# 2alaaa/distributed-llm-scheduler

Hardware: AMD Instinct MI355X
Metric: DAG makespan (ms) + tasks completed under mem cap, GPT-2 DAG at 1/2/4/8 MI355X (lower is better)
Workload: dtype bf16

## Files before the change

csrc/kernels/gemm_glds_impl.h:

```cpp
#pragma once
#include <cstdlib>
#include <type_traits>
#include "common.h"
#include "kernels.h"
#include "gemm_glds_cfgs.h"

#ifndef DLS_STAMP
#define DLS_STAMP(k)
#endif

namespace {

__device__ __forceinline__ int kslice_count(int K, int kslice) { return K / kslice; }

template <int N>
__device__ __forceinline__ void wait_vm() {
  asm volatile("s_waitcnt vmcnt(%0)" ::"n"(N) : "memory");
}
template <int PW, int A>
__device__ __forceinline__ void wait_tiles(int ahead) {
  if constexpr (A == 0) {
    wait_vm<0>();
  } else {
    if (ahead >= A) wait_vm<PW * A>();
    else wait_tiles<PW, A - 1>(ahead);
  }
}
__device__ __forceinline__ void raw_barrier() { asm volatile("s_barrier" ::: "memory"); }
template <class T>
__device__ __forceinline__ void consume_from_here(T& x) {
  asm volatile("" : "+v"(x));
}
template <bool WAIT_LDS_ONLY>
__device__ __forceinline__ void epi_barrier() {
  if constexpr (WAIT_LDS_ONLY) asm volatile("s_waitcnt lgkmcnt(0)\n\ts_barrier" ::: "memory");
  else __syncthreads();
}

template <int BM_, int BN_, int WM_, int WN_, int STAGES_, int PRIO_ = 0, int BXS_ = 0, int KG_ = 1, int RING_ = 0,
          int OCC_ = 1>
struct Cfg {
  static constexpr int BM = BM_, BN = BN_, WM = WM_, WN = WN_, STAGES = STAGES_, PRIO = PRIO_, BXS = BXS_;
  static constexpr int KG = KG_, RING = RING_, OCC = OCC_;
  static constexpr int BK = 64, CH = 8;
  static constexpr int NW = WM * WN, T = 64 * NW * KG;
  static constexpr int WTM = BM / WM, WTN = BN / WN, FM = WTM / 16, FN = WTN / 16;
  static constexpr bool HALF_FRAGS = FM + FN > 12;
  static constexpr int ROWS = BM + BN, INSTR = ROWS / 8, PW = (INSTR + NW - 1) / NW;
  static constexpr int SUB = ROWS * CH;
  static constexpr int STAGE = SUB * KG;
  static constexpr int SA = STAGES, SB = STAGES + BXS;
  static constexpr int PWA = (BM / 8 + NW - 1) / NW, PWB = (BN / 8 + NW - 1) / NW;
  static constexpr bool EVEN = INSTR % NW == 0, EVEN_A = (BM / 8) % NW == 0, EVEN_B = (BN / 8) % NW == 0;
  static constexpr int A_STAGE = BM * CH, B_STAGE = BN * CH;
  static constexpr int LDS_UNITS = BXS ? SA * A_STAGE + SB * B_STAGE : STAGES * STAGE;
  static_assert(BM % 8 == 0 && BN % 8 == 0, "DMA pieces are 8 rows");
  static_assert(FM >= 1 && FN >= 1, "wave tile too small");
  static_assert(PW * (STAGES - 2) <= 63, "vmcnt range");
  static_assert(!BXS || (SA - 2) * PWA + (SA - 1) * PWB <= 63, "vmcnt range (split rings)");
  static_assert(STAGES >= 2 && STAGES <= 8, "stages");
  static_assert(LDS_UNITS * 16 <= 163840, "LDS budget");
  static_assert(KG == 1 || (BXS == 0 && PRIO == 0), "K groups use the joint ring");
  static_assert(KG == 1 || (KG - 1) * NW * 64 * FM * FN * 16 <= LDS_UNITS * 16, "K-group reduction must fit the LDS");
  static constexpr bool EPI_BATCH = FM * FN <= 4;
// ... 647 lines not shown
          float csv[8] = {0.f, 0.f, 0.f, 0.f, 0.f, 0.f, 0.f, 0.f};
          if (bias) {
            uint32_t w[8];
            if (pre_bvec) {
#pragma unroll
              for (int h = 0; h < 2; ++h) {
                consume_from_here(o_bv[h]);
                const uint32_t p0 = o_bv[h][0], p1 = o_bv[h][1];
                w[4 * h + 0] = p0 << 16;
                w[4 * h + 1] = p0 & 0xffff0000u;
                w[4 * h + 2] = p1 << 16;
                w[4 * h + 3] = p1 & 0xffff0000u;
              }
            } else {
#pragma unroll
              for (int e = 0; e < 8; ++e) {
                consume_from_here(o_bs[e]);
                w[e] = o_bs[e] << 16;
              }
            }
#pragma unroll
            for (int e = 0; e < 8; ++e) bv[e] = col + e < N ? __uint_as_float(w[e]) : 0.f;
          }
          if constexpr (LNM) {
#pragma unroll
            for (int h = 0; h < 2; ++h) consume_from_here(o_cs[h]);
#pragma unroll
            for (int e = 0; e < 8; ++e) csv[e] = col + e < N ? __uint_as_float(o_cs[e >> 2][e & 3]) : 0.f;
          }
          float v[8];
#pragma unroll
          for (int e = 0; e < 8; ++e) {
            const float x = e < 4 ? lo[e & 3] : hi[e & 3];
            if constexpr (LNM) v[e] = act_c<ACT>(ln_rs1 * (x - ln_mu1 * csv[e]) + bv[e]);
            else v[e] = act_c<ACT>(alpha * x + bv[e]);
          }
          if constexpr (ROPE) {
            rope_pairs<4>(v, row, col, rope);
            rope_pairs<4>(v + 4, row, col + 4, rope);
          }
#pragma unroll
          for (int e = 0; e < 8; ++e) o[e] = f2bf(v[e]);
        };
        per_epilogue(finish);
        if (pre_res) consume_from_here(o_r);
        store_segment(o, rl, cc, o_r);
      }
      DLS_STAMP(3)
      return;
    }
  }
  if constexpr (C::EPI_BATCH) {
    if (part == nullptr && act != ACT_SWIGLU) request_operands();
  }
  if constexpr (C::KG > 2) {
    constexpr int REG = C::NW * C::FM * C::FN * 64;
    epi_barrier<C::EPI_BATCH>();
    f32x4* red = reinterpret_cast<f32x4*>(smem);
    if (kgrp != 0) {
#pragma unroll
      for (int i = 0; i < C::FM; ++i)
#pragma unroll
        for (int j = 0; j < C::FN; ++j)
          red[(kgrp - 1) * REG + ((i * C::FN + j) * C::NW + wq) * 64 + lane] = acc[i][j];
    }
    epi_barrier<C::EPI_BATCH>();
    if (kgrp == 0) {
#pragma unroll
// ... 612 lines not shown
  using type = Cfg<224, 256, 2, 4, 2, 0, 1>;
};
template <>
struct TallTile<C33> {
  using type = C14;
};

template <class C>
void grouped(const GemmArgs& a, int n_groups, const int* offsets, const unsigned long long* w_ptrs,
             const unsigned long long* c_ptrs, hipStream_t s, const int* a_rows) {
  static const int w_stream = [] {
    const char* e = std::getenv("DLS_EXPERT_NT");
    return e && e[0] == '0' ? 0 : 1;
  }();
  const char* pe = std::getenv("DLS_EXPERT_PAIRS");
  const int pairs = pe && *pe ? std::atoi(pe) : 2;
  const int pair = a.grouped_shared ? 0 : pairs;
  const char* xe = std::getenv("DLS_EXPERT_XCD");
  const bool xcd = xe && *xe == '1' && !a.grouped_shared && pair != 1;
  const char* te = std::getenv("DLS_EXPERT_TALL");
  const bool tall = !(te && *te == '0') && !a.grouped_shared;
  const Epi ep{a.rope, nullptr, nullptr, nullptr, w_ptrs, c_ptrs,
               (a.grouped_shared ? 8 : ((size_t)a.M * a.lda * 2 < (1ull << 31) ? w_stream : 0)) |
                   (pair == 1 ? 16 : pair == 2 ? 32 : pair == 3 ? 64 : 0) | (xcd ? 128 : 0) | (tall ? 256 : 0)};
  const int tiles_n = (a.N + C::BN - 1) / C::BN;
  const int blocks = pair == 1 ? (n_groups * tiles_n + 7) / 8 * 16 : pair >= 2 ? 2 * n_groups * tiles_n
                                                                               : n_groups * tiles_n;
  hipLaunchKernelGGL((gemm_glds_kernel<C, 0, 3>), dim3(blocks), dim3(C::T), 0, s, (const bf16*)a.A, a.lda,
                     nullptr, a.ldw, (bf16*)a.C, a.ldc, nullptr, nullptr, 0,
                     const_cast<float*>(reinterpret_cast<const float*>(a_rows)), a.M, a.N, a.K, a.act, a.alpha,
                     n_groups, tiles_n, 1, a.K, nullptr, 0, 1e-5f, offsets, a.compact_rows, ep);
}

template <int W_, int S_>
struct PrivCfg {
  static constexpr int W = W_, S = S_, BM = 32, BN = 48, BK = 64, CH = 8, FM = 2, FN = 3;
  static constexpr int T = 64 * W, PW = (BM + BN) / 8;
  static constexpr int SLOT = (BM + BN) * CH;
  static constexpr int RING = S * SLOT, LDS_UNITS = W * RING;
  static constexpr int REG = FM * FN * 64;
  static_assert(S >= 1 && PW * (S - 1) <= 63, "vmcnt range");
  static_assert(LDS_UNITS * 16 <= 163840 && T <= 1024, "LDS budget, block size");
  static_assert(REG <= RING, "a wave's fragment region lies inside its own ring");
  static_assert(T >= BM * 8, "one 16-byte output segment per storing thread");
};

template <class P>
__device__ __forceinline__ void mainloop_private(bf16x8* ring, const bf16* __restrict__ A, int lda,
                                                 const bf16* __restrict__ W, int ldw, int M, int N, int m0, int n0,
                                                 int kbeg, int nk, int lane, f32x4 (&acc)[P::FM][P::FN]) {
  const bf16* src[P::PW];
#pragma unroll
  for (int j = 0; j < P::PW; ++j) {
    const int row = 8 * j + (lane >> 3);
    const int kofs = kbeg + ((lane & 7) ^ (row & 7)) * 8;
    src[j] = row < P::BM ? A + (size_t)min(m0 + row, M - 1) * lda + kofs
                         : W + (size_t)min(n0 + row - P::BM, N - 1) * ldw + kofs;
  }
  auto issue = [&](int kt, bf16x8* slot) {
#pragma unroll
    for (int j = 0; j < P::PW; ++j)
      __builtin_amdgcn_global_load_lds((const void*)(src[j] + kt * P::BK),
                                       (__attribute__((address_space(3))) void*)(slot + j * 64), 16, 0, 0);
  };
#pragma unroll
  for (int s = 0; s < P::S; ++s)
    if (s < nk) issue(s, ring + s * P::SLOT);
  int sl = 0;
  for (int kt = 0; kt < nk; ++kt) {
    wait_tiles<P::PW, P::S - 1>(min(P::S - 1, nk - 1 - kt));
    bf16x8* slot = ring + sl * P::SLOT;
    const bf16x8* sA = slot;
    const bf16x8* sB = slot + P::BM * P::CH;
    bf16x8 af[2][P::FM], bw[2][P::FN];
#pragma unroll
    for (int kk = 0; kk < 2; ++kk) {
      const int chunk = kk * 4 + (lane >> 4);
#pragma unroll
      for (int j = 0; j < P::FN; ++j) {
        const int row = j * 16 + (lane & 15);
        bw[kk][j] = sB[row * P::CH + (chunk ^ (row & 7))];
      }
#pragma unroll
      for (int i = 0; i < P::FM; ++i) {
        const int row = i * 16 + (lane & 15);
        af[kk][i] = sA[row * P::CH + (chunk ^ (row & 7))];
      }
    }
    __builtin_amdgcn_sched_barrier(0);
    asm volatile("s_waitcnt lgkmcnt(0)" ::: "memory");
    __builtin_amdgcn_sched_barrier(0);
    if (kt + P::S < nk) issue(kt + P::S, slot);
    __builtin_amdgcn_sched_barrier(0);
#pragma unroll
    for (int kk = 0; kk < 2; ++kk)
#pragma unroll
      for (int i = 0; i < P::FM; ++i)
#pragma unroll
        for (int j = 0; j < P::FN; ++j) acc[i][j] = mfma16x16x32(bw[kk][j], af[kk][i], acc[i][j]);
    sl = sl + 1 == P::S ? 0 : sl + 1;
  }
}

template <class P, int SPOL>
__global__ __launch_bounds__(P::T, 1) void gemm_private_kernel(const bf16* __restrict__ A, int lda,
                                                               const bf16* __restrict__ W, int ldw,
                                                               bf16* __restrict__ Cp, int ldc,
                                                               const bf16* __restrict__ bias,
                                                               const bf16* __restrict__ R, int ldr,
                                                               float* __restrict__ stats_out, int M, int N, int K,
                                                               float alpha, int tiles_m) {
  __shared__ bf16x8 smem[P::LDS_UNITS];
  const int tid = threadIdx.x, lane = tid & 63;
  const int wave = __builtin_amdgcn_readfirstlane(tid >> 6);
  const int tile = xcd_remap(blockIdx.x, gridDim.x);
  const int m0 = (tile % tiles_m) * P::BM, n0 = (tile / tiles_m) * P::BN;
  DLS_STAMP(0)
  const int nk = K / (P::BK * P::W);
  bf16x8* ring = smem + wave * P::RING;
  f32x4 acc[P::FM][P::FN];
#pragma unroll
  for (int i = 0; i < P::FM; ++i)
#pragma unroll
    for (int j = 0; j < P::FN; ++j) acc[i][j] = f32x4{0.f, 0.f, 0.f, 0.f};
  mainloop_private<P>(ring, A, lda, W, ldw, M, N, m0, n0, wave * nk * P::BK, nk, lane, acc);
  DLS_STAMP(1)
  constexpr int BNC = P::BN / 8, BNP = 8;
  const bool own = tid < P::BM * BNP;
  const int rl = tid / BNP, cc = tid % BNP;
  const int row = m0 + rl, col = n0 + cc * 8;
  const bool pre_bvec = ((reinterpret_cast<uintptr_t>(bias) & 7) | (N & 3)) == 0;
  const bool v16 = ((reinterpret_cast<uintptr_t>(Cp) | ((uintptr_t)ldc * 2)) & 15) == 0 &&
                   (!R || ((reinterpret_cast<uintptr_t>(R) | ((uintptr_t)ldr * 2)) & 15) == 0);
  const bool pre_res = R != nullptr && N >= 8 && v16 && ((size_t)(M + P::BM) * ldr * 2 < (1ull << 31));
  u32x2 o_bv[2];
  u32x4 o_r;
  if (own) {
    constexpr int kRaw = 0x00020000;
    if (bias && pre_bvec) {
      const auto rs = __builtin_amdgcn_make_buffer_rsrc(const_cast<bf16*>(bias), 0, N * 2, kRaw);
#pragma unroll
      for (int h = 0; h < 2; ++h) o_bv[h] = __builtin_amdgcn_raw_buffer_load_b64(rs, col * 2 + h * 8, 0, 0);
    }
    if (pre_res) {
// ... 90 lines not shown
        s2 += __shfl_xor(s2, o_, 64);
      }
      if (cc == 0 && row < M) {
        atomicAdd(stats_out + 2 * row, s1);
        atomicAdd(stats_out + 2 * row + 1, s2);
      }
    }
  }
  DLS_STAMP(3)
}

inline bool private_takes(int waves, const GemmArgs& a, int splitk, bool folded_norm, bool ranged) {
  return waves > 0 && a.K > 0 && a.K % (64 * waves) == 0 && splitk <= 1 && !folded_norm && !ranged &&
         a.act == ACT_NONE && a.rope.cols == 0 && !a.ext_stats;
}

template <int W_, int S_>
void launch_private(const GemmArgs& a, hipStream_t s) {
  using P = PrivCfg<W_, S_>;
  const int tiles_m = (a.M + P::BM - 1) / P::BM, tiles_n = (a.N + P::BN - 1) / P::BN;
  dim3 grid(tiles_m * tiles_n), block(P::T);
#define DLS_PK(POL_)                                                                                               \
  hipLaunchKernelGGL((gemm_private_kernel<P, POL_>), grid, block, 0, s, (const bf16*)a.A, a.lda, (const bf16*)a.W, \
                     a.ldw, (bf16*)a.C, a.ldc, (const bf16*)a.bias, (const bf16*)a.R, a.ldr, a.stats_out, a.M, a.N, \
                     a.K, a.alpha, tiles_m)
  switch ((size_t)a.M * a.ldc * 2 < (1ull << 31) ? a.stream_pol & 7 : 0) {
    case 2: case 3: DLS_PK(kPolStream); break;
    case 4: case 5: DLS_PK(kPolWT); break;
    default: DLS_PK(0);
  }
#undef DLS_PK
}

}

#define DLS_GLDS_DEFINE(ID)                                                                                     \
  bool glds_launch_cfg##ID(const GemmArgs& a, int splitk, float* ws, hipStream_t s, const float* ln_colsum,     \
                           int ln_mode, float ln_eps, const int* rows, bool persist) {                          \
    return launch<C##ID>(a, splitk, ws, s, ln_colsum, ln_mode, ln_eps, rows, persist);                          \
  }                                                                                                             \
  void glds_grouped_cfg##ID(const GemmArgs& a, int n_groups, const int* offsets, const unsigned long long* w_ptrs, \
                            const unsigned long long* c_ptrs, hipStream_t s, const int* a_rows) {               \
    grouped<C##ID>(a, n_groups, offsets, w_ptrs, c_ptrs, s, a_rows);                                            \
  }
```

csrc/kernels/gemm_private.hip:

```cpp
#include "gemm_glds_impl.h"

namespace {
constexpr int kWaves[kGemmPrivateCount] = {8, 4, 6, 12};
}

int gemm_private_waves(int cfg) {
  return cfg >= kGemmPrivate && cfg < kGemmPrivate + kGemmPrivateCount ? kWaves[cfg - kGemmPrivate] : 0;
}

bool gemm_private_takes(const GemmArgs& a, int cfg, int splitk, bool folded_norm, bool ranged) {
  return private_takes(gemm_private_waves(cfg), a, splitk, folded_norm, ranged);
}

bool launch_gemm_private(const GemmArgs& a, int cfg, hipStream_t s) {
  if (!gemm_private_takes(a, cfg, 1, false, false)) return false;
  switch (cfg - kGemmPrivate) {
    case 0: launch_private<8, 2>(a, s); break;
    case 1: launch_private<4, 3>(a, s); break;
    case 2: launch_private<6, 2>(a, s); break;
    default: launch_private<12, 1>(a, s); break;
  }
  return true;
}
```

csrc/kernels/kernels.h:

```cpp
#pragma once

#include <hip/hip_runtime_api.h>
#include <stdint.h>

constexpr int kActSwiglu = 4;

struct RopeArgs {
  const float* cos = nullptr;
  const float* sin = nullptr;
  int S = 1, D = 2, cols = 0;
};

struct GemmArgs {
  const void* A;
  int lda;
  const void* W;
  int ldw;
  void* C;
  int ldc;
  const void* bias;
  const void* R;
  int ldr;
  int M, N, K;
  int act;
// ... 11 lines not shown
  int norm_mode = 0;
  float norm_eps = 1e-5f;
  int ldn = 0;
  int stream_pol = 0;
};

struct Epi {
  RopeArgs rope;
  float* stats_out;
  const float* ext_stats;
  int* tile_sem = nullptr;
  const unsigned long long* grp_w = nullptr;
  const unsigned long long* grp_c = nullptr;
  int w_stream = 0;
};

int gemm_pick_config(int M, int N, int K);
void launch_gemm_bf16(const GemmArgs& a, hipStream_t s);

int gemm_glds_num_configs();
int gemm_glds_kstep(int cfg);
void gemm_glds_tile(int cfg, int* bm, int* bn);
int gemm_glds_resolve(int cfg, int act, bool ln_in);
constexpr int kGemmPersist = 64;
void gemm_glds_pick(int M, int N, int K, int* cfg, int* splitk);
size_t gemm_glds_workspace_bytes(int M, int N, int splitk);
bool launch_gemm_glds(const GemmArgs& a, int cfg, int splitk, void* workspace, hipStream_t s,
                      const float* ln_colsum = nullptr, int ln_mode = 0, float ln_eps = 1e-5f,
                      const int* rows = nullptr);
constexpr int kGemmPrivate = 120, kGemmPrivateCount = 4;
int gemm_private_waves(int cfg);
bool gemm_private_takes(const GemmArgs& a, int cfg, int splitk, bool folded_norm, bool ranged);
bool launch_gemm_private(const GemmArgs& a, int cfg, hipStream_t s);

void launch_gemm_glds_grouped(const GemmArgs& a, int cfg, int n_groups, const int* offsets,
                              const unsigned long long* w_ptrs, const unsigned long long* c_ptrs, hipStream_t s,
                              const int* a_rows = nullptr);

struct GemmGroupedSkinnyArgs {
  const void* A;
  int lda;
  int a_total;
  const int* a_rows;
  const int* offsets;
  const unsigned long long* w_ptrs;
  const unsigned long long* c_ptrs;
  void* C;
  int ldc;
  int compact_rows;
  int R, N, K;
  int act;
  int n_groups;
};
bool gemm_grouped_skinny_takes(int N, int K, int act);
void launch_gemm_grouped_skinny(const GemmGroupedSkinnyArgs& a, hipStream_t s);

constexpr int kSkinnyMaxRows = 16;
struct GemmSkinnyArgs {
  const void* A;
  int lda;
  const void* W;
  int ldw;
  void* C;
  int ldc;
  const void* bias;
  const void* R;
// ... 350 lines not shown
```

csrc/kernels/ops_binding.cpp:

```cpp
#include <cstdlib>

#include <torch/extension.h>
#include <c10/hip/HIPStream.h>

#include "kernels.h"

namespace {

hipStream_t cur_stream() { return c10::hip::getCurrentHIPStream().stream(); }

constexpr int64_t kSemPool = 1 << 20;
int64_t sem_next[64];
int* split_k_counters(const at::Tensor& like, int64_t n) {
  static at::Tensor* pool = new at::Tensor[64];
  int64_t* next = sem_next;
  const int d = like.get_device();
  TORCH_CHECK(d >= 0 && d < 64 && n <= kSemPool, "split-K counters");
  if (!pool[d].defined()) pool[d] = at::zeros({kSemPool}, like.options().dtype(at::kInt));
  n = (n + 63) / 64 * 64;
  if (next[d] + n > kSemPool) next[d] = 0;
  int* p = pool[d].data_ptr<int>() + next[d];
  next[d] += n;
  return p;
}
// ... 10 lines not shown
  const int old = g_fixup_max_slices;
  if (n > 0) g_fixup_max_slices = (int)std::min<int64_t>(n, 1 << 30);
  return old;
}

void check_bf16(const at::Tensor& t, const char* name) {
  TORCH_CHECK(t.is_cuda(), name, " must be a GPU tensor");
  TORCH_CHECK(t.scalar_type() == at::kBFloat16, name, " must be bfloat16");
}

void check_rows(const at::Tensor& t, const char* name) {
  TORCH_CHECK(t.dim() == 2, name, " must be 2-D");
  TORCH_CHECK(t.stride(1) == 1, name, " must have contiguous rows");
  TORCH_CHECK(t.stride(0) % 8 == 0, name, " row stride must be a multiple of 8 elements");
  TORCH_CHECK(reinterpret_cast<uintptr_t>(t.data_ptr()) % 16 == 0, name, " must be 16-byte aligned");
}

at::Tensor as2d(const at::Tensor& t) { return t.dim() == 2 ? t : t.reshape({-1, t.size(-1)}); }

constexpr int64_t kRegStage = 100;

at::Tensor gemm(const at::Tensor& a_in, const at::Tensor& w, const c10::optional<at::Tensor>& bias,
                const c10::optional<at::Tensor>& residual, int64_t act, double alpha,
                const c10::optional<at::Tensor>& out, int64_t config, int64_t splitk,
                const c10::optional<at::Tensor>& ln_colsum, int64_t ln_mode, double ln_eps,
                const c10::optional<at::Tensor>& rows, bool compact_rows,
                const c10::optional<at::Tensor>& rope_cos, const c10::optional<at::Tensor>& rope_sin, int64_t rope_S,
                int64_t rope_D, int64_t rope_cols, const c10::optional<at::Tensor>& stats_out,
                const c10::optional<at::Tensor>& ext_stats, const c10::optional<at::Tensor>& norm_out,
                const c10::optional<at::Tensor>& norm_w, const c10::optional<at::Tensor>& norm_b, int64_t norm_mode,
                double norm_eps, int64_t stream_pol) {
  check_bf16(a_in, "A");
  check_bf16(w, "W");
  const bool priv = gemm_private_waves((int)config) != 0;
  TORCH_CHECK(config < kRegStage + 4 || priv, "unknown GEMM config ", config, " (register-staged configs are ",
              kRegStage, "..", kRegStage + 3, ", wave-private rings ", kGemmPrivate, "..",
              kGemmPrivate + kGemmPrivateCount - 1, ")");
  at::Tensor a = as2d(a_in);
  check_rows(a, "A");
  check_rows(w, "W");
  const int64_t M = a.size(0), K = a.size(1), N = w.size(0);
  const bool swiglu = act == kActSwiglu;
  const int64_t NO = swiglu ? N / 2 : N;
  TORCH_CHECK(w.size(1) == K, "W must be [N][K] with K = ", K, ", got ", w.sizes());
  TORCH_CHECK(K % 8 == 0, "K must be a multiple of 8");
  TORCH_CHECK(!swiglu || (N % 32 == 0 && K % 64 == 0 && !residual.has_value()),
              "SwiGLU epilogue needs N % 32 == 0, K % 64 == 0 and no residual");
  at::Tensor c;
  if (out.has_value()) {
    c = as2d(*out);
    check_bf16(c, "out");
    TORCH_CHECK((c.size(0) == M || (compact_rows && c.size(0) <= M)) && c.size(1) == NO && c.stride(1) == 1,
                "out must be [M][N_out] (or fewer rows with compact_rows)");
  } else {
    c = at::empty({M, NO}, a.options());
  }
  const void* bptr = nullptr;
  if (bias.has_value()) {
    check_bf16(*bias, "bias");
    TORCH_CHECK(bias->is_contiguous() && bias->numel() == N, "bias must be contiguous [N]");
    bptr = bias->data_ptr();
  }
  const void* rptr = nullptr;
  int ldr = 0;
  if (residual.has_value()) {
    at::Tensor r = as2d(*residual);
    check_bf16(r, "residual");
    TORCH_CHECK(r.size(0) == M && r.size(1) == N && r.stride(1) == 1, "residual must be [M][N]");
    rptr = r.data_ptr();
    ldr = (int)r.stride(0);
// ... 35 lines not shown
    if (norm_mode == 2)
      launch_rmsnorm(c.data_ptr(), nullptr, nullptr, g.norm_w, y_n.data_ptr(), (int)M, (int)N, (float)norm_eps,
                     cur_stream());
    else
      launch_layernorm(c.data_ptr(), nullptr, nullptr, g.norm_w, g.norm_b, y_n.data_ptr(), (int)M, (int)N,
                       (float)norm_eps, cur_stream());
  };
  TORCH_CHECK(!compact_rows || (rows.has_value() && !residual.has_value()), "compact_rows needs rows and no residual");
  auto check_stats = [&](const at::Tensor& t, const char* name) {
    TORCH_CHECK(t.is_cuda() && t.scalar_type() == at::kFloat && t.is_contiguous() && t.numel() == 2 * M, name,
                " must be a contiguous fp32 [M][2] GPU tensor");
  };
  if (stats_out.has_value()) {
    check_stats(*stats_out, "stats_out");
    TORCH_CHECK(!swiglu && !rows.has_value(), "row statistics are emitted by plain (non-SwiGLU, full-row) GEMMs");
    g.stats_out = stats_out->data_ptr<float>();
  }
  if (ext_stats.has_value()) {
    check_stats(*ext_stats, "ext_stats");
    TORCH_CHECK(ln_mode != 0, "ext_stats needs ln_mode (1 LayerNorm, 2 RMSNorm) and ln_colsum");
    g.ext_stats = ext_stats->data_ptr<float>();
  }
  if (rope_cols > 0) {
    TORCH_CHECK(rope_cos.has_value() && rope_sin.has_value() && rope_cos->scalar_type() == at::kFloat &&
                    rope_sin->scalar_type() == at::kFloat && rope_cos->is_contiguous() && rope_sin->is_contiguous() &&
                    rope_cos->is_cuda() && rope_sin->is_cuda() &&
                    rope_cos->numel() >= rope_S * rope_D / 2 && rope_sin->numel() >= rope_S * rope_D / 2,
                "RoPE epilogue: cos/sin fp32 [S][D/2]");
    TORCH_CHECK(rope_D % 4 == 0 && rope_cols % rope_D == 0 && rope_cols <= N && !swiglu && K % 64 == 0 &&
                    !rows.has_value() && act == 0,
                "RoPE epilogue: D % 4 == 0, whole heads, LDS-DMA kernel, no activation / SwiGLU / row range");
    g.rope = RopeArgs{rope_cos->data_ptr<float>(), rope_sin->data_ptr<float>(), (int)rope_S, (int)rope_D,
                      (int)rope_cols};
    if (config >= kRegStage && !priv) config = -1;
  }
  const bool glds_ok = (K % 64 == 0);
  const float* csp = nullptr;
  if (ln_mode != 0) {
    TORCH_CHECK(glds_ok, "fused norm-GEMM needs K % 64 == 0");
    TORCH_CHECK(ln_colsum.has_value() && ln_colsum->scalar_type() == at::kFloat && ln_colsum->is_contiguous() &&
                    ln_colsum->numel() == N,
                "fused norm-GEMM needs fp32 ln_colsum [N]");
    csp = ln_colsum->data_ptr<float>();
  }
  if (priv) {
    TORCH_CHECK(!compact_rows && gemm_private_takes(g, (int)config, (int)splitk, ln_mode != 0, rowp != nullptr),
                "GEMM config ", config, " (wave-private rings, ", gemm_private_waves((int)config),
                " waves) takes plain launches only: K % ", 64 * gemm_private_waves((int)config),
                " == 0, no activation, folded norm, RoPE, SwiGLU, split-K or row range");
    TORCH_CHECK(launch_gemm_private(g, (int)config, cur_stream()), "GEMM config ", config, " refused the launch");
    post_norm(false);
    return c;
  }
  if (ln_mode != 0 || swiglu || rowp || stats_out.has_value()) {
    TORCH_CHECK(glds_ok, "this epilogue needs the LDS-DMA kernel (K % 64 == 0)");
    if (config >= kRegStage) config = -1;
  }
  if (config >= kRegStage || !glds_ok) {
    g.config = config >= kRegStage ? (int)(config - kRegStage) : -1;
    launch_gemm_bf16(g, cur_stream());
    post_norm(false);
    return c;
  }
  int cfg = (int)config, sk = (int)splitk;
  if (cfg < 0 || sk <= 0) {
    int acfg, ask;
    gemm_glds_pick((int)M, (int)N, (int)K, &acfg, &ask);
    if (cfg < 0) cfg = acfg;
    if (sk <= 0) sk = ask;
  }
  TORCH_CHECK((cfg & (kGemmPersist - 1)) < gemm_glds_num_configs() && cfg < 2 * kGemmPersist, "unknown GEMM config ", cfg);
  TORCH_CHECK(K % gemm_glds_kstep(cfg) == 0, "GEMM config ", cfg, " needs K % ", gemm_glds_kstep(cfg), " == 0");
  const bool split_ok = (N % 8 == 0) && (c.stride(0) % 8 == 0) && (ldr % 8 == 0) &&
                        K % (gemm_glds_kstep(cfg) * sk) == 0 &&
                        (!swiglu || N % 32 == 0);
  if (!split_ok || (ln_mode != 0 && !ext_stats.has_value())) sk = 1;
  at::Tensor ws;
  if (sk > 1) {
    ws = at::empty({(int64_t)gemm_glds_workspace_bytes((int)M, (int)N, sk) / 4}, a.options().dtype(at::kFloat));
    if (kSplitKFixup && sk <= g_fixup_max_slices && !rowp && !norm_out.has_value()) {
      int bm, bn;
      gemm_glds_tile(gemm_glds_resolve(cfg, (int)act, false), &bm, &bn);
      g.tile_sem = split_k_counters(a, (M + bm - 1) / bm * ((N + bn - 1) / bn));
// ... 1478 lines not shown
        py::arg("stats_out") = py::none(), py::arg("ext_stats") = py::none(), py::arg("norm_out") = py::none(),
        py::arg("norm_w") = py::none(), py::arg("norm_b") = py::none(), py::arg("norm_mode") = 0,
        py::arg("norm_eps") = 1e-5, py::arg("stream_pol") = 0);
  m.def("gemm_w8", &gemm_w8, py::arg("a"), py::arg("wq"), py::arg("scale"), py::arg("bias") = py::none(),
        py::arg("residual") = py::none(), py::arg("act") = 0, py::arg("alpha") = 1.0, py::arg("out") = py::none(),
        py::arg("config") = -1, py::arg("splitk") = 0, py::arg("store_pol") = 0, py::arg("workspace") = py::none());
  m.def("gemm_w8_num_configs", &gemm_w8_num_configs);
  m.def("gemm_w8_pick", [](int M, int N, int K) {
    int c, s;
    gemm_w8_pick(M, N, K, &c, &s);
    return std::make_pair(c, s);
  });
  m.def("gemm_grouped_w8", &gemm_grouped_w8, py::arg("x"), py::arg("weights"), py::arg("scales"), py::arg("w_ptrs"),
        py::arg("s_ptrs"), py::arg("offsets"), py::arg("act") = 0, py::arg("out") = py::none(),
        py::arg("outs") = std::vector<at::Tensor>{}, py::arg("out_ptrs") = py::none(), py::arg("config") = -1,
        py::arg("rows_hint") = 0, py::arg("a_rows") = py::none(), py::arg("shared_weights") = false,
        py::arg("store_pol") = 0);
  m.def("gemm_w8_grouped_num_configs", &gemm_w8_grouped_num_configs);
  m.def("gemm_w8_grouped_tile_rows", &gemm_w8_grouped_tile_rows);
  m.def("gemm_w8_grouped_pick", &gemm_w8_grouped_pick);
  m.def("gemm_grouped_w4a8", &gemm_grouped_w4a8, py::arg("xq"), py::arg("xscale"), py::arg("weights"),
        py::arg("scales"), py::arg("w_ptrs"), py::arg("s_ptrs"), py::arg("offsets"), py::arg("act") = 0,
        py::arg("out") = py::none(), py::arg("outs") = std::vector<at::Tensor>{}, py::arg("out_ptrs") = py::none(),
        py::arg("config") = -1, py::arg("rows_hint") = 0, py::arg("a_rows") = py::none(),
        py::arg("shared_weights") = false, py::arg("store_pol") = 0);
  m.def("gemm_w4a8_grouped_num_configs", &gemm_w4a8_grouped_num_configs);
  m.def("gemm_w4a8_grouped_tile_rows", &gemm_w4a8_grouped_tile_rows);
  m.def("gemm_w4a8_grouped_pick", &gemm_w4a8_grouped_pick);
  m.attr("REGSTAGE") = kRegStage;
  m.attr("PERSIST") = kGemmPersist;
  m.attr("PRIVATE") = kGemmPrivate;
  m.attr("PRIVATE_COUNT") = kGemmPrivateCount;
  m.def("gemm_private_waves", &gemm_private_waves);
  m.def("gemm_pick_config", &gemm_pick_config);
  m.def("gemm_glds_num_configs", &gemm_glds_num_configs);
  m.def("gemm_glds_kstep", &gemm_glds_kstep);
  m.def("gemm_glds_tile", [](int64_t cfg) {
    int bm, bn;
    gemm_glds_tile((int)cfg, &bm, &bn);
    return std::make_tuple((int64_t)bm, (int64_t)bn);
  });
  m.def("_split_k_cursor", &split_k_cursor);
  m.def("gemm_glds_pick", [](int M, int N, int K) {
    int c, s;
    gemm_glds_pick(M, N, K, &c, &s);
    return std::make_pair(c, s);
  });
  m.def("attention", &attention, py::arg("q"), py::arg("k"), py::arg("v"), py::arg("B"), py::arg("S"),
        py::arg("n_head"), py::arg("n_kv_head"), py::arg("head_dim"), py::arg("causal") = true,
        py::arg("scale") = 0.125, py::arg("out") = py::none(), py::arg("variant") = 0, py::arg("Sq") = 0,
        py::arg("q_off") = 0, py::arg("flags") = 0);
  m.def("kv_append", &kv_append, py::arg("k_new"), py::arg("v_new"), py::arg("k_cache"), py::arg("v_cache"),
        py::arg("pos"), py::arg("T"), py::arg("k_scale") = py::none(), py::arg("v_scale") = py::none());
  m.def("attention_decode_sizes", &attention_decode_sizes, py::arg("B"), py::arg("T"), py::arg("C"),
        py::arg("n_head"), py::arg("n_kv_head"), py::arg("head_dim"), py::arg("chunk") = 0);
  m.def("attention_decode_chunk", [](int64_t B, int64_t C, int64_t n_kv_head, int64_t head_dim) {
    return (int64_t)attn_decode_chunk((int)B, (int)C, (int)n_kv_head, (int)head_dim);
  });
  m.def("attention_decode", &attention_decode, py::arg("q"), py::arg("k_cache"), py::arg("v_cache"), py::arg("pos"),
        py::arg("T"), py::arg("n_head"), py::arg("n_kv_head"), py::arg("head_dim"), py::arg("scale"),
        py::arg("part"), py::arg("cnt"), py::arg("out") = py::none(), py::arg("chunk") = 0,
        py::arg("k_scale") = py::none(), py::arg("v_scale") = py::none());
  m.def("gemm_fixup_max_slices", &gemm_fixup_max_slices, py::arg("n") = 0);
  m.def("kv_dequantize_rows", &kv_dequantize_rows, py::arg("cache"), py::arg("scale"), py::arg("pos"), py::arg("T"),
        py::arg("out"));
  m.def("attention_chunk_variant", &attention_chunk_variant, py::arg("B"), py::arg("T"), py::arg("n_head"),
// ... 80 lines not shown
```

distributed_llm_scheduler_amd/ops/__init__.py:

```python
from __future__ import annotations

import math
import os
import threading
from typing import Optional, Tuple

import torch
import torch.nn.functional as F

from . import tuning

ACT = {None: 0, "none": 0, "gelu": 1, "gelu_tanh": 1, "silu": 2, "relu": 3, "swiglu": 4}
SWIGLU = 4
SWIGLU_BLOCK = 16
LMHEAD_POL = int(os.environ.get("DLS_LMHEAD_POL", "3"))
LMHEAD_MIN_N = 32000
WEIGHT_NT_MB = float(os.environ.get("DLS_WEIGHT_NT_MB", "0"))
ACT_POL = int(os.environ.get("DLS_ACT_POL", "4"))
ACT_POL_MODEL = {"mixtral-8x7b": 0}
_ACT_POL_SET = "DLS_ACT_POL" in os.environ
ATTN_FLAGS = int(os.environ.get("DLS_ATTN_FLAGS", "0"))
ATTN_VARIANT = int(os.environ.get("DLS_ATTN_VARIANT", "0"))


# ... 168 lines not shown
    return dict(norm_out=y, norm_w=nw, norm_b=nb if kind == "layernorm" else None,
                norm_mode=1 if kind == "layernorm" else 2, norm_eps=float(eps))


def _post_norm_ref(src, post_norm):
    y, nw, nb, kind, eps = post_norm
    s2 = src.reshape(-1, src.shape[-1])
    r = ref_layernorm(s2, nw, nb, eps) if kind == "layernorm" else ref_rmsnorm(s2, nw, eps)
    y.view(r.shape).copy_(r)


def linear(x, w, bias=None, act=None, residual=None, alpha=1.0, out=None, rows=None, rows_hint=None,
           compact=False, rope=None, stats_out=None, post_norm=None):
    a = ACT[act] if not isinstance(act, int) else act
    n_out = w.shape[0] // 2 if a == SWIGLU else w.shape[0]
    if _gpu(x):
        shp = x.shape[:-1] + (n_out,)
        M = x.numel() // x.shape[-1]
        cfg, sk = tuning.lookup(rows_hint or M, w.shape[0], w.shape[1], tuning.tag(a, rows is not None))
        if cfg == tuning.LIB:
            if tuning.VENDOR and a == 0 and residual is None and rows is None and rope is None \
                    and stats_out is None and post_norm is None:
                x2 = x.reshape(M, x.shape[-1])
                o2 = out.view(M, n_out) if out is not None else torch.empty(M, n_out, dtype=x.dtype, device=x.device)
                if bias is not None:
                    torch.addmm(bias, x2, w.t(), beta=1.0, alpha=float(alpha), out=o2)
                else:
                    torch.mm(x2, w.t(), out=o2)
                    if alpha != 1.0:
                        o2.mul_(alpha)
                return o2.view(shp) if out is None else out
            cfg, sk = tuning.lookup_fused(rows_hint or M, w.shape[0], w.shape[1], tuning.tag(a, rows is not None))
        cfg, sk = tuning.resolve_private((cfg, sk), w.shape[1], a, rows is not None, rope is not None)
        rc, rs_, rS, rD, rcols = rope if rope is not None else (None, None, 1, 2, 0)
        y = ext().gemm(x, w, bias, residual, a, float(alpha), out, cfg, sk, None, 0, 1e-5, rows, bool(compact),
                       rc, rs_, int(rS), int(rD), int(rcols), stats_out, None,
                       stream_pol=_stream_pol(w.shape[0], w.shape[1]) if rows is None else 0,
                       **(_post_norm_args(post_norm) if post_norm is not None else {}))
        return y.view(shp) if out is None else out
    if rows is not None:
        r0, r1 = (int(v) for v in rows.tolist())
        if out is None:
            out = torch.zeros(x.shape[:-1] + (n_out,), dtype=x.dtype)
        res = residual[r0:r1] if residual is not None else None
        o2 = out.reshape(-1, out.shape[-1])
        if compact:
            n = min(r1 - r0, o2.shape[0])
            o2[:n] = ref_linear(x[r0:r0 + n], w, bias, act, None, alpha)
        else:
            o2[r0:r1] = ref_linear(x[r0:r1], w, bias, act, res, alpha)
        return out
    y = ref_linear(x, w, bias, act, residual, alpha, rope=rope)
    if out is not None:
        out.copy_(y)
        y = out
    if post_norm is not None:
        _post_norm_ref(y, post_norm)
    return y


def quantize_fp8(w):
    from ..models.params import quantize_fp8 as _q
    return _q(w)


def dequantize_fp8(q, scale, dtype=torch.bfloat16):
# ... 158 lines not shown


def derive_norm_gemm(w, ln_w, ln_b=None, bias=None):
    wf = w.float()
    wd = (wf * ln_w.float()[None, :]).to(w.dtype)
    cs = wd.float().sum(1).contiguous()
    b = torch.zeros(w.shape[0], device=w.device) if bias is None else bias.float()
    if ln_b is not None:
        b = b + (wf * ln_b.float()[None, :]).sum(1)
    return wd, cs, b.to(w.dtype).contiguous()


def linear_norm(x, w_derived, colsum, bias_derived, mode, eps=1e-5, act=None, residual=None, out=None, rope=None,
                ext_stats=None):
    m = {"layernorm": 1, "rmsnorm": 2}[mode]
    a = ACT[act] if not isinstance(act, int) else act
    shp = x.shape[:-1] + (w_derived.shape[0] // 2 if a == SWIGLU else w_derived.shape[0],)
    M, N, K = x.numel() // x.shape[-1], w_derived.shape[0], w_derived.shape[1]
    split = tuning.col_split(M, N, K, tuning.tag(a)) if ext_stats is not None and rope is None and a != SWIGLU \
        else None
    if split:
        if out is None:
            out = torch.empty(shp, dtype=x.dtype, device=x.device)
        o2 = out.view(M, N)
        r2 = residual.reshape(M, N) if residual is not None else None
        pol = _stream_pol(N, K)
        for n0, n1, c, k in split:
            ext().gemm(x, w_derived[n0:n1], bias_derived[n0:n1] if bias_derived is not None else None,
                       r2[:, n0:n1] if r2 is not None else None, a, 1.0, o2[:, n0:n1], int(c), int(k),
                       colsum[n0:n1], m, float(eps), None, False, None, None, 1, 2, 0, None, ext_stats,
                       stream_pol=pol)
        return out
    cfg, sk = tuning.resolve_private(tuning.lookup_fused(M, N, K, tuning.tag(a)), K, a, folded=True)
    if ext_stats is None:
        sk = 1
        if 0 <= cfg < tuning.REGSTAGE and tuning.kstep(cfg) != 64:
            cfg = next((int(c) for c, _ in tuning.runner_ups(M, N, K, tuning.tag(a), 8)
                        if 0 <= c < tuning.REGSTAGE and tuning.kstep(c) == 64), -1)
    rc, rs_, rS, rD, rcols = rope if rope is not None else (None, None, 1, 2, 0)
    pol = _stream_pol(N, K)
    y = ext().gemm(x, w_derived, bias_derived, residual, a, 1.0, out, cfg if cfg < tuning.REGSTAGE else -1, sk, colsum,
                   m, float(eps), None, False, rc, rs_, int(rS), int(rD), int(rcols), None, ext_stats,
                   stream_pol=pol)
    return y.view(shp) if out is None else out



SKINNY_ROWS_LIMIT = 16
SKINNY_WAVES = (4, 8, 16)
SKINNY_MAX_ROWS = 2
SKINNY_LMHEAD = True
_NORM_MODE = {"layernorm": 1, "rmsnorm": 2, 1: 1, 2: 2}


def skinny_waves(N: int, K: int, act=None) -> int:
    a = ACT[act] if not isinstance(act, int) else act
    strips = N // 32 if a == SWIGLU else (N + 15) // 16
    nk = (K + 63) // 64
    if a == SWIGLU:
        return 4
    return 16 if strips >= 4096 and nk >= 32 else 8


def skinny_refusal(M, N, K, act=None, rope=None, norm=None, waves=None, lda=None, ldw=None) -> Optional[str]:
    try:
        a = ACT[act] if not isinstance(act, int) else act
    except KeyError:
        return f"unknown activation {act!r}"
    lda, ldw = (K if lda is None else lda), (K if ldw is None else ldw)
    if not 1 <= M <= SKINNY_ROWS_LIMIT:
        return f"M = {M}: the kernel takes 1..{SKINNY_ROWS_LIMIT} rows"
    if N < 1 or K < 32 or K % 32:
        return f"N = {N}, K = {K}: N >= 1 and K a positive multiple of 32"
    if lda % 8 or ldw % 8 or lda < K or ldw < K:
# ... 873 lines not shown
```

distributed_llm_scheduler_amd/ops/tuning.py:

```python
from __future__ import annotations

import json
import os
import statistics
import threading
from typing import Dict, Iterable, Optional, Tuple

import torch

_PATH = os.environ.get("DLS_GEMM_TUNING") or os.path.join(os.path.dirname(os.path.abspath(__file__)),
                                                          "gemm_tuning.json")
_lock = threading.Lock()
_table: Optional[Dict[str, Tuple[int, int]]] = None
_cands: Dict[str, list] = {}
_refined: Dict[str, bool] = {}
_col_splits: Dict[str, list] = {}
_overrides: Dict[str, Dict[str, Tuple[int, int]]] = {}
_model: Optional[str] = None
REGSTAGE = 100
PERSIST = 64
LIB = 200
VENDOR = os.environ.get("DLS_ALLOW_VENDOR_GEMM", "0") == "1"
PRIVATE = 120
PRIVATE_WAVES = {120: 8, 121: 4, 122: 6, 123: 12}
PRIVATE_FALLBACK = (45, 1)


def private_takes(cfg: int, K: int, sk: int = 1, act: int = 0, ranged: bool = False, rope: bool = False,
                  folded: bool = False) -> bool:
    w = PRIVATE_WAVES.get(cfg, 0)
    return w > 0 and K > 0 and K % (64 * w) == 0 and sk <= 1 and act == 0 and not (ranged or rope or folded)


def resolve_private(choice: Tuple[int, int], K: int, act: int = 0, ranged: bool = False, rope: bool = False,
                    folded: bool = False) -> Tuple[int, int]:
    cfg, sk = choice
    if cfg not in PRIVATE_WAVES:
        return choice
    return (cfg, 1) if private_takes(cfg, K, sk, act, ranged, rope, folded) else PRIVATE_FALLBACK


def _key(M: int, N: int, K: int, tg: str = "") -> str:
    return f"{M}x{N}x{K}{tg}"


def tag(act: int = 0, ranged: bool = False) -> str:
    return ("s" if act == 4 else "") + ("r" if ranged else "")


def table() -> Dict[str, Tuple[int, int]]:
    global _table
    with _lock:
        if _table is None:
            _table = {}
            if os.path.exists(_PATH):
                try:
                    with open(_PATH) as f:
                        doc = json.load(f)
                    _table = {k: tuple(v) for k, v in doc.get("gemm", {}).items()}
                    _cands.update({k: [tuple(c) for c in v] for k, v in doc.get("candidates", {}).items()})
                    _refined.update(doc.get("refined", {}))
                    _col_splits.update({k: [tuple(x) for x in v] for k, v in doc.get("col_splits", {}).items()})
                    _overrides.update({m: {k: tuple(v) for k, v in t.items()}
                                       for m, t in doc.get("model_overrides", {}).items()})
                except (OSError, ValueError):
                    _table = {}
        return _table


def set_model(name: Optional[str]) -> None:
    global _model
    _model = name
# ... 218 lines not shown
```

Baseline: 0.5363.

## Add 64-row wave-private split-K GEMM kernel with folded-norm epilogue

Adds a new wave-private-ring GEMM kernel that works on 64-row tiles with 80 or 96 columns and reduces the per-wave K partial sums through LDS. Its epilogue folds LayerNorm/RMSNorm from external stats and applies an optional GELU. Config ids 130-133 are wired into the binding, the tuning resolver and the fused-norm Python path. The kernel only runs when the tuning table selects these ids, and nothing in this change adds such entries, so default behaviour may be unchanged.

```diff
diff --git a/csrc/kernels/gemm_glds_impl.h b/csrc/kernels/gemm_glds_impl.h
--- a/csrc/kernels/gemm_glds_impl.h
+++ b/csrc/kernels/gemm_glds_impl.h
@@ -30,6 +30,11 @@
 template <class T>
 __device__ __forceinline__ void consume_from_here(T& x) {
   asm volatile("" : "+v"(x));
+}
+template <int ACT, bool LNM>
+__device__ __forceinline__ float finish_value(float x, float alpha, float rs, float mu, float cs, float b) {
+  if constexpr (LNM) return act_c<ACT>(rs * (x - mu * cs) + b);
+  else return act_c<ACT>(alpha * x + b);
 }
 template <bool WAIT_LDS_ONLY>
 __device__ __forceinline__ void epi_barrier() {
@@ -743,8 +748,7 @@
 #pragma unroll
           for (int e = 0; e < 8; ++e) {
             const float x = e < 4 ? lo[e & 3] : hi[e & 3];
-            if constexpr (LNM) v[e] = act_c<ACT>(ln_rs1 * (x - ln_mu1 * csv[e]) + bv[e]);
-            else v[e] = act_c<ACT>(alpha * x + bv[e]);
+            v[e] = finish_value<ACT, LNM>(x, alpha, ln_rs1, ln_mu1, csv[e], bv[e]);
           }
           if constexpr (ROPE) {
             rope_pairs<4>(v, row, col, rope);
@@ -1423,18 +1427,20 @@
                      n_groups, tiles_n, 1, a.K, nullptr, 0, 1e-5f, offsets, a.compact_rows, ep);
 }
 
-template <int W_, int S_>
-struct PrivCfg {
-  static constexpr int W = W_, S = S_, BM = 32, BN = 48, BK = 64, CH = 8, FM = 2, FN = 3;
+template <int BM_, int BN_, int W_, int S_>
+struct PrivTile {
+  static constexpr int W = W_, S = S_, BM = BM_, BN = BN_, BK = 64, CH = 8, FM = BM / 16, FN = BN / 16;
   static constexpr int T = 64 * W, PW = (BM + BN) / 8;
   static constexpr int SLOT = (BM + BN) * CH;
   static constexpr int RING = S * SLOT, LDS_UNITS = W * RING;
   static constexpr int REG = FM * FN * 64;
+  static_assert(BM % 16 == 0 && BN % 16 == 0, "whole 16 x 16 fragments");
   static_assert(S >= 1 && PW * (S - 1) <= 63, "vmcnt range");
   static_assert(LDS_UNITS * 16 <= 163840 && T <= 1024, "LDS budget, block size");
   static_assert(REG <= RING, "a wave's fragment region lies inside its own ring");
-  static_assert(T >= BM * 8, "one 16-byte output segment per storing thread");
 };
+template <int W_, int S_>
+using PrivCfg = PrivTile<32, 48, W_, S_>;
 
 template <class P>
 __device__ __forceinline__ void mainloop_private(bf16x8* ring, const bf16* __restrict__ A, int lda,
@@ -1501,6 +1507,7 @@
                                                                const bf16* __restrict__ R, int ldr,
                                                                float* __restrict__ stats_out, int M, int N, int K,
                                                                float alpha, int tiles_m) {
+  static_assert(P::T >= P::BM * 8, "one 16-byte output segment per storing thread");
   __shared__ bf16x8 smem[P::LDS_UNITS];
   const int tid = threadIdx.x, lane = tid & 63;
   const int wave = __builtin_amdgcn_readfirstlane(tid >> 6);
@@ -1657,6 +1664,185 @@
 #undef DLS_PK
 }
 
+template <class P, int SPOL>
+__global__ __launch_bounds__(P::T, 1) void gemm_private_wide_kernel(const bf16* __restrict__ A,
+                                                                    const bf16* __restrict__ W, bf16* __restrict__ Cp,
+                                                                    const bf16* __restrict__ bias,
+                                                                    const float* __restrict__ ln_colsum,
+                                                                    const float* __restrict__ ext_stats, int lda,
+                                                                    int ldw, int ldc, int M, int N, int K, int tiles_m,
+                                                                    int ln_mode, int act, float ln_eps) {
+  constexpr int BNC = P::BN / 8, NQ = (BNC + 3) / 4;
+  constexpr int SEGS = P::BM * NQ * 4, NPASS = SEGS / P::T;
+  static_assert(SEGS % P::T == 0, "whole passes: no thread without a segment");
+  __shared__ bf16x8 smem[P::LDS_UNITS];
+  const int tid = threadIdx.x, lane = tid & 63;
+  const int wave = __builtin_amdgcn_readfirstlane(tid >> 6);
+  const int tile = xcd_remap(blockIdx.x, gridDim.x);
+  const int m0 = (tile % tiles_m) * P::BM, n0 = (tile / tiles_m) * P::BN;
+  DLS_STAMP(0)
+  const int nk = K / (P::BK * P::W);
+  bf16x8* ring = smem + wave * P::RING;
+  f32x4 acc[P::FM][P::FN];
+#pragma unroll
+  for (int i = 0; i < P::FM; ++i)
+#pragma unroll
+    for (int j = 0; j < P::FN; ++j) acc[i][j] = f32x4{0.f, 0.f, 0.f, 0.f};
+  mainloop_private<P>(ring, A, lda, W, ldw, M, N, m0, n0, wave * nk * P::BK, nk, lane, acc);
+  DLS_STAMP(1)
+  auto seg_row = [&](int p) { const int q = tid + p * P::T; return (q >> 4) / NQ * 4 + ((q >> 2) & 3); };
+  auto seg_chunk = [&](int p) { const int q = tid + p * P::T; return (q >> 4) % NQ * 4 + (q & 3); };
+  const bool pre_bvec = ((reinterpret_cast<uintptr_t>(bias) & 7) | (N & 3)) == 0;
+  const bool pre_cvec = ((reinterpret_cast<uintptr_t>(ln_colsum) & 15) | (N & 3)) == 0;
+  const bool v16 = ((reinterpret_cast<uintptr_t>(Cp) | ((uintptr_t)ldc * 2)) & 15) == 0;
+  u32x2 o_st[NPASS];
+  u32x2 o_bv[NPASS][2];
+  u32x4 o_cs[NPASS][2];
+  {
+    constexpr int kRaw = 0x00020000;
+    const auto rst = __builtin_amdgcn_make_buffer_rsrc(const_cast<float*>(ext_stats), 0, M * 8, kRaw);
+#pragma unroll
+    for (int p = 0; p < NPASS; ++p) o_st[p] = __builtin_amdgcn_raw_buffer_load_b64(rst, (m0 + seg_row(p)) * 8, 0, 0);
+    if (bias && pre_bvec) {
+      const auto rs = __builtin_amdgcn_make_buffer_rsrc(const_cast<bf16*>(bias), 0, N * 2, kRaw);
+#pragma unroll
+      for (int p = 0; p < NPASS; ++p)
+#pragma unroll
+        for (int h = 0; h < 2; ++h)
+          o_bv[p][h] = __builtin_amdgcn_raw_buffer_load_b64(rs, (n0 + seg_chunk(p) * 8) * 2 + h * 8, 0, 0);
+    }
+    if (pre_cvec) {
+      const auto rs = __builtin_amdgcn_make_buffer_rsrc(const_cast<float*>(ln_colsum), 0, N * 4, kRaw);
+#pragma unroll
+      for (int p = 0; p < NPASS; ++p)
+#pragma unroll
+        for (int h = 0; h < 2; ++h)
+          o_cs[p][h] = __builtin_amdgcn_raw_buffer_load_b128(rs, (n0 + seg_chunk(p) * 8) * 4 + h * 16, 0, 0);
+    }
+  }
+  f32x4* reg = reinterpret_cast<f32x4*>(ring);
+#pragma unroll
+  for (int i = 0; i < P::FM; ++i)
+#pragma unroll
+    for (int j = 0; j < P::FN; ++j) {
+      const int cl = j * 16 + (lane >> 4) * 4;
+      reg[(i * P::FN + j) * 64 + (lane & 48) + ((lane & 15) ^ (((cl >> 3) & 3) << 2))] = acc[i][j];
+    }
+  epi_barrier<true>();
+  DLS_STAMP(7)
+  const f32x4* red = reinterpret_cast<const f32x4*>(smem);
+  f32x4 lo[NPASS], hi[NPASS];
+#pragma unroll
+  for (int p = 0; p < NPASS; ++p) {
+    const int rl = seg_row(p);
+    const int ccr = min(seg_chunk(p), BNC - 1), cl0 = ccr * 8;
+    const int rec = ((rl / 16) * P::FN + cl0 / 16) * 64 + (cl0 & 8) * 4 + ((rl & 15) ^ ((ccr & 3) << 2));
+    f32x4 part_lo[P::W], part_hi[P::W];
+#pragma unroll
+    for (int w = 0; w < P::W; ++w) {
+      part_lo[w] = red[w * P::RING + rec];
+      part_hi[w] = red[w * P::RING + rec + 16];
+    }
+    lo[p] = part_lo[0], hi[p] = part_hi[0];
+#pragma unroll
+    for (int w = 1; w < P::W; ++w) {
+      lo[p] += part_lo[w];
+      hi[p] += part_hi[w];
+    }
+  }
+  const float inv_k = 1.0f / (float)K;
+  float rs[NPASS], mu[NPASS], bv[NPASS][8], csv[NPASS][8];
+#pragma unroll
+  for (int p = 0; p < NPASS; ++p) {
+    const int col = n0 + seg_chunk(p) * 8;
+    consume_from_here(o_st[p]);
+    const float a = __uint_as_float(o_st[p][0]), q = __uint_as_float(o_st[p][1]);
+    mu[p] = ln_mode == 1 ? a * inv_k : 0.f;
+    rs[p] = rsqrtf(fmaxf(q * inv_k - mu[p] * mu[p], 0.f) + ln_eps);
+#pragma unroll
+    for (int e = 0; e < 8; ++e) bv[p][e] = csv[p][e] = 0.f;
+    if (bias) {
+      if (pre_bvec) {
+        uint32_t w[8];
+#pragma unroll
+        for (int h = 0; h < 2; ++h) {
+          consume_from_here(o_bv[p][h]);
+          const uint32_t p0 = o_bv[p][h][0], p1 = o_bv[p][h][1];
+          w[4 * h + 0] = p0 << 16;
+          w[4 * h + 1] = p0 & 0xffff0000u;
+          w[4 * h + 2] = p1 << 16;
+          w[4 * h + 3] = p1 & 0xffff0000u;
+        }
+#pragma unroll
+        for (int e = 0; e < 8; ++e) bv[p][e] = col + e < N ? __uint_as_float(w[e]) : 0.f;
+      } else {
+#pragma unroll
+        for (int e = 0; e < 8; ++e)
+          if (col + e < N) bv[p][e] = bf2f(bias[col + e]);
+      }
+    }
+    if (pre_cvec) {
+#pragma unroll
+      for (int h = 0; h < 2; ++h) consume_from_here(o_cs[p][h]);
+#pragma unroll
+      for (int e = 0; e < 8; ++e) csv[p][e] = col + e < N ? __uint_as_float(o_cs[p][e >> 2][e & 3]) : 0.f;
+    } else {
+#pragma unroll
+      for (int e = 0; e < 8; ++e)
+        if (col + e < N) csv[p][e] = ln_colsum[col + e];
+    }
+  }
+  bf16x8 seg[NPASS];
+  auto finish = [&](auto act_tag) {
+    constexpr int ACT = decltype(act_tag)::value;
+#pragma unroll
+    for (int p = 0; p < NPASS; ++p)
+#pragma unroll
+      for (int e = 0; e < 8; ++e)
+        seg[p][e] = f2bf(finish_value<ACT, true>(e < 4 ? lo[p][e & 3] : hi[p][e & 3], 1.f, rs[p], mu[p], csv[p][e],
+                                                 bv[p][e]));
+  };
+  if (act == ACT_GELU_TANH) finish(std::integral_constant<int, ACT_GELU_TANH>{});
+  else finish(std::integral_constant<int, ACT_NONE>{});
+#pragma unroll
+  for (int p = 0; p < NPASS; ++p) {
+    const int cc = seg_chunk(p), row = m0 + seg_row(p), col = n0 + cc * 8;
+    if (cc < BNC && row < M && col < N) {
+      if (v16 && col + 8 <= N) {
+        store16_pol<SPOL>(Cp, ((size_t)row * ldc + col) * 2, *reinterpret_cast<const u32x4*>(&seg[p]));
+      } else {
+#pragma unroll
+        for (int e = 0; e < 8; ++e)
+          if (col + e < N) Cp[(size_t)row * ldc + col + e] = seg[p][e];
+      }
+    }
+  }
+  DLS_STAMP(3)
+}
+
+inline bool private_wide_takes(int waves, const GemmArgs& a, int splitk, int ln_mode, bool ranged) {
+  return waves > 0 && a.K > 0 && a.K % (64 * waves) == 0 && splitk <= 1 && (ln_mode == 1 || ln_mode == 2) &&
+         a.ext_stats && !ranged && (a.act == ACT_NONE || a.act == ACT_GELU_TANH) && a.rope.cols == 0 && !a.R &&
+         !a.stats_out;
+}
+
+template <int BM_, int BN_, int W_, int S_>
+void launch_private_wide(const GemmArgs& a, const float* ln_colsum, int ln_mode, float ln_eps, hipStream_t s) {
+  using P = PrivTile<BM_, BN_, W_, S_>;
+  const int tiles_m = (a.M + P::BM - 1) / P::BM, tiles_n = (a.N + P::BN - 1) / P::BN;
+  dim3 grid(tiles_m * tiles_n), block(P::T);
+#define DLS_PK(POL_)                                                                                              \
+  hipLaunchKernelGGL((gemm_private_wide_kernel<P, POL_>), grid, block, 0, s, (const bf16*)a.A, (const bf16*)a.W, \
+                     (bf16*)a.C, (const bf16*)a.bias, ln_colsum, a.ext_stats, a.lda, a.ldw, a.ldc, a.M, a.N, a.K, \
+                     tiles_m, ln_mode, a.act, ln_eps)
+  switch ((size_t)a.M * a.ldc * 2 < (1ull << 31) ? a.stream_pol & 7 : 0) {
+    case 2: case 3: DLS_PK(kPolStream); break;
+    case 4: case 5: DLS_PK(kPolWT); break;
+    default: DLS_PK(0);
+  }
+#undef DLS_PK
+}
+
 }
 
 #define DLS_GLDS_DEFINE(ID)                                                                                     \
diff --git a/csrc/kernels/gemm_private.hip b/csrc/kernels/gemm_private.hip
--- a/csrc/kernels/gemm_private.hip
+++ b/csrc/kernels/gemm_private.hip
@@ -22,3 +22,25 @@
   }
   return true;
 }
+
+int gemm_private_wide_waves(int cfg) {
+  return cfg >= kGemmPrivateWide && cfg < kGemmPrivateWide + kGemmPrivateWideCount
+             ? kGemmPrivateWideCfgs[cfg - kGemmPrivateWide].waves
+             : 0;
+}
+
+bool gemm_private_wide_takes(const GemmArgs& a, int cfg, int splitk, int ln_mode, bool ranged) {
+  return private_wide_takes(gemm_private_wide_waves(cfg), a, splitk, ln_mode, ranged);
+}
+
+bool launch_gemm_private_wide(const GemmArgs& a, int cfg, const float* ln_colsum, int ln_mode, float ln_eps,
+                              hipStream_t s) {
+  if (!ln_colsum || !gemm_private_wide_takes(a, cfg, 1, ln_mode, false)) return false;
+  switch (cfg - kGemmPrivateWide) {
+    case 0: launch_private_wide<64, 96, 4, 2>(a, ln_colsum, ln_mode, ln_eps, s); break;
+    case 1: launch_private_wide<64, 96, 3, 2>(a, ln_colsum, ln_mode, ln_eps, s); break;
+    case 2: launch_private_wide<64, 80, 4, 2>(a, ln_colsum, ln_mode, ln_eps, s); break;
+    default: launch_private_wide<64, 80, 3, 2>(a, ln_colsum, ln_mode, ln_eps, s); break;
+  }
+  return true;
+}
diff --git a/csrc/kernels/kernels.h b/csrc/kernels/kernels.h
--- a/csrc/kernels/kernels.h
+++ b/csrc/kernels/kernels.h
@@ -67,6 +67,15 @@
 int gemm_private_waves(int cfg);
 bool gemm_private_takes(const GemmArgs& a, int cfg, int splitk, bool folded_norm, bool ranged);
 bool launch_gemm_private(const GemmArgs& a, int cfg, hipStream_t s);
+constexpr int kGemmPrivateWide = 130, kGemmPrivateWideCount = 4;
+struct GemmPrivateWideCfg {
+  int bm, bn, waves, slots;
+};
+constexpr GemmPrivateWideCfg kGemmPrivateWideCfgs[kGemmPrivateWideCount] = {{64, 96, 4, 2}, {64, 96, 3, 2}, {64, 80, 4, 2}, {64, 80, 3, 2}};
+int gemm_private_wide_waves(int cfg);
+bool gemm_private_wide_takes(const GemmArgs& a, int cfg, int splitk, int ln_mode, bool ranged);
+bool launch_gemm_private_wide(const GemmArgs& a, int cfg, const float* ln_colsum, int ln_mode, float ln_eps,
+                              hipStream_t s);
 
 void launch_gemm_glds_grouped(const GemmArgs& a, int cfg, int n_groups, const int* offsets,
                               const unsigned long long* w_ptrs, const unsigned long long* c_ptrs, hipStream_t s,
diff --git a/csrc/kernels/ops_binding.cpp b/csrc/kernels/ops_binding.cpp
--- a/csrc/kernels/ops_binding.cpp
+++ b/csrc/kernels/ops_binding.cpp
@@ -66,10 +66,12 @@
                 double norm_eps, int64_t stream_pol) {
   check_bf16(a_in, "A");
   check_bf16(w, "W");
+  const bool wide = gemm_private_wide_waves((int)config) != 0;
   const bool priv = gemm_private_waves((int)config) != 0;
-  TORCH_CHECK(config < kRegStage + 4 || priv, "unknown GEMM config ", config, " (register-staged configs are ",
-              kRegStage, "..", kRegStage + 3, ", wave-private rings ", kGemmPrivate, "..",
-              kGemmPrivate + kGemmPrivateCount - 1, ")");
+  TORCH_CHECK(config < kRegStage + 4 || priv || wide, "unknown GEMM config ", config,
+              " (register-staged configs are ", kRegStage, "..", kRegStage + 3, ", wave-private rings ", kGemmPrivate,
+              "..", kGemmPrivate + kGemmPrivateCount - 1, " and ", kGemmPrivateWide, "..",
+              kGemmPrivateWide + kGemmPrivateWideCount - 1, ")");
   at::Tensor a = as2d(a_in);
   check_rows(a, "A");
   check_rows(w, "W");
@@ -171,7 +173,7 @@
                 "RoPE epilogue: D % 4 == 0, whole heads, LDS-DMA kernel, no activation / SwiGLU / row range");
     g.rope = RopeArgs{rope_cos->data_ptr<float>(), rope_sin->data_ptr<float>(), (int)rope_S, (int)rope_D,
                       (int)rope_cols};
-    if (config >= kRegStage && !priv) config = -1;
+    if (config >= kRegStage && !priv && !wide) config = -1;
   }
   const bool glds_ok = (K % 64 == 0);
   const float* csp = nullptr;
@@ -188,6 +190,17 @@
                 " waves) takes plain launches only: K % ", 64 * gemm_private_waves((int)config),
                 " == 0, no activation, folded norm, RoPE, SwiGLU, split-K or row range");
     TORCH_CHECK(launch_gemm_private(g, (int)config, cur_stream()), "GEMM config ", config, " refused the launch");
+    post_norm(false);
+    return c;
+  }
+  if (wide) {
+    TORCH_CHECK(!compact_rows && gemm_private_wide_takes(g, (int)config, (int)splitk, (int)ln_mode, rowp != nullptr),
+                "GEMM config ", config, " (wave-private rings on 64-row tiles, ", gemm_private_wide_waves((int)config),
+                " waves) takes folded-norm launches with ext_stats only: K % ",
+                64 * gemm_private_wide_waves((int)config),
+                " == 0, no activation or GeLU, no RoPE, SwiGLU, split-K, row range, residual or stats_out");
+    TORCH_CHECK(launch_gemm_private_wide(g, (int)config, csp, (int)ln_mode, (float)ln_eps, cur_stream()),
+                "GEMM config ", config, " refused the launch");
     post_norm(false);
     return c;
   }
@@ -1732,6 +1745,13 @@
   m.attr("PRIVATE") = kGemmPrivate;
   m.attr("PRIVATE_COUNT") = kGemmPrivateCount;
   m.def("gemm_private_waves", &gemm_private_waves);
+  m.attr("PRIVATE_WIDE") = kGemmPrivateWide;
+  m.attr("PRIVATE_WIDE_COUNT") = kGemmPrivateWideCount;
+  m.def("gemm_private_wide_cfg", [](int64_t cfg) {
+    TORCH_CHECK(gemm_private_wide_waves((int)cfg) != 0, "GEMM config ", cfg, " is not a 64-row wave-private id");
+    const GemmPrivateWideCfg& w = kGemmPrivateWideCfgs[cfg - kGemmPrivateWide];
+    return std::make_tuple(w.bm, w.bn, w.waves, w.slots);
+  });
   m.def("gemm_pick_config", &gemm_pick_config);
   m.def("gemm_glds_num_configs", &gemm_glds_num_configs);
   m.def("gemm_glds_kstep", &gemm_glds_kstep);
diff --git a/distributed_llm_scheduler_amd/ops/__init__.py b/distributed_llm_scheduler_amd/ops/__init__.py
--- a/distributed_llm_scheduler_amd/ops/__init__.py
+++ b/distributed_llm_scheduler_amd/ops/__init__.py
@@ -224,6 +224,7 @@
                 return o2.view(shp) if out is None else out
             cfg, sk = tuning.lookup_fused(rows_hint or M, w.shape[0], w.shape[1], tuning.tag(a, rows is not None))
         cfg, sk = tuning.resolve_private((cfg, sk), w.shape[1], a, rows is not None, rope is not None)
+        cfg, sk = tuning.resolve_private_wide((cfg, sk), w.shape[1], a, rows is not None, rope is not None)
         rc, rs_, rS, rD, rcols = rope if rope is not None else (None, None, 1, 2, 0)
         y = ext().gemm(x, w, bias, residual, a, float(alpha), out, cfg, sk, None, 0, 1e-5, rows, bool(compact),
                        rc, rs_, int(rS), int(rD), int(rcols), stats_out, None,
@@ -448,6 +449,8 @@
                        stream_pol=pol)
         return out
     cfg, sk = tuning.resolve_private(tuning.lookup_fused(M, N, K, tuning.tag(a)), K, a, folded=True)
+    cfg, sk = tuning.resolve_private_wide((cfg, sk), K, a, rope=rope is not None, folded=True,
+                                          ext_stats=ext_stats is not None, residual=residual is not None)
     if ext_stats is None:
         sk = 1
         if 0 <= cfg < tuning.REGSTAGE and tuning.kstep(cfg) != 64:
@@ -455,7 +458,9 @@
                         if 0 <= c < tuning.REGSTAGE and tuning.kstep(c) == 64), -1)
     rc, rs_, rS, rD, rcols = rope if rope is not None else (None, None, 1, 2, 0)
     pol = _stream_pol(N, K)
-    y = ext().gemm(x, w_derived, bias_derived, residual, a, 1.0, out, cfg if cfg < tuning.REGSTAGE else -1, sk, colsum,
+    if cfg >= tuning.REGSTAGE and cfg not in tuning.PRIVATE_WIDE_CFGS:
+        cfg = -1
+    y = ext().gemm(x, w_derived, bias_derived, residual, a, 1.0, out, cfg, sk, colsum,
                    m, float(eps), None, False, rc, rs_, int(rS), int(rD), int(rcols), None, ext_stats,
                    stream_pol=pol)
     return y.view(shp) if out is None else out
diff --git a/distributed_llm_scheduler_amd/ops/tuning.py b/distributed_llm_scheduler_amd/ops/tuning.py
--- a/distributed_llm_scheduler_amd/ops/tuning.py
+++ b/distributed_llm_scheduler_amd/ops/tuning.py
@@ -38,6 +38,30 @@
     if cfg not in PRIVATE_WAVES:
         return choice
     return (cfg, 1) if private_takes(cfg, K, sk, act, ranged, rope, folded) else PRIVATE_FALLBACK
+
+
+PRIVATE_WIDE = 130
+PRIVATE_WIDE_CFGS = {130: (64, 96, 4, 2), 131: (64, 96, 3, 2), 132: (64, 80, 4, 2), 133: (64, 80, 3, 2)}
+PRIVATE_WIDE_FALLBACK = (17, 1)
+
+
+def private_wide_takes(cfg: int, K: int, sk: int = 1, act: int = 0, ranged: bool = False, rope: bool = False,
+                       folded: bool = False, ext_stats: bool = False, residual: bool = False,
+                       stats_out: bool = False) -> bool:
+    w = PRIVATE_WIDE_CFGS.get(cfg, (0, 0, 0, 0))[2]
+    return (w > 0 and K > 0 and K % (64 * w) == 0 and sk <= 1 and act in (0, 1) and folded and ext_stats
+            and not (ranged or rope or residual or stats_out))
+
+
+def resolve_private_wide(choice: Tuple[int, int], K: int, act: int = 0, ranged: bool = False, rope: bool = False,
+                         folded: bool = False, ext_stats: bool = False, residual: bool = False,
+                         stats_out: bool = False) -> Tuple[int, int]:
+    cfg, sk = choice
+    if cfg not in PRIVATE_WIDE_CFGS:
+        return choice
+    if private_wide_takes(cfg, K, sk, act, ranged, rope, folded, ext_stats, residual, stats_out):
+        return (cfg, 1)
+    return PRIVATE_WIDE_FALLBACK
 
 
 def _key(M: int, N: int, K: int, tg: str = "") -> str:
```

Result: faster. 0.5273 (median of 6 runs) (-1.7%).
